# HerreraKrachTeichmann/NJODE

Measured on AMD Instinct MI355X. Metric: paths/sec (training step) on 20k Black-Scholes, 100 steps, higher is better.
Workload: dtype f32; 1 GPU; BlackScholes 20000 paths/GPU x 100 grid steps, every rank's paths as one batch, hidden_size=10, 3x(50,50) tanh nets, dropout 0.1, train step = plan+fwd+bwd+Adam; global_batch=20000, n_obs_rows=199470, euler_steps_per_batch=1820212, params=10071, parallelism=dp1

## Files before the change

include/njode_hip.h:

```cpp
#ifndef NJODE_HIP_H
#define NJODE_HIP_H

#include <stddef.h>
#include <stdint.h>

#ifdef __cplusplus
extern "C" {
#endif

typedef struct ihipStream_t* njodeStream_t;

#define NJODE_OK 0
#define NJODE_E_UNSUPPORTED 1
#define NJODE_E_BADARG 2
#define NJODE_E_WORKSPACE 3
#define NJODE_E_HIP 4

#define NJODE_ACT_TANH 0
#define NJODE_ACT_RELU 1

#define NJODE_F_MASKED 0x1
#define NJODE_F_INPUT_CURRENT_T 0x2
#define NJODE_F_RESIDUAL 0x4
#define NJODE_F_LOSS_EASY 0x8
// ... 64 lines not shown

int njode_workspace_bytes(const NjodeDims* dims, int32_t batch_size, int32_t n_obs,
                          int32_t n_times, int32_t n_steps, int32_t call_flags,
                          size_t* out);

int njode_plan_flush(void);
int njode_plan_bytes(const NjodeDims* dims, int32_t batch_size, int32_t n_obs,
                     int32_t n_times, int32_t n_steps, int32_t call_flags, size_t* out);
int njode_plan_f32(const NjodeDims* dims, const NjodeBatch* batch, const NjodeSchedule* sched,
                   int32_t call_flags, void* plan, size_t plan_bytes, njodeStream_t stream);


int njode_forward_f32(const NjodeDims* dims, const float* params,
                      const NjodeBatch* batch, const NjodeSchedule* sched,
                      int32_t call_flags, float weight, float dropout_p,
                      uint64_t seed, float* hT, float* loss, float* path_h,
                      float* path_y, void* workspace, size_t workspace_bytes,
                      njodeStream_t stream);

int njode_backward_f32(const NjodeDims* dims, const float* params,
                       const NjodeBatch* batch, const NjodeSchedule* sched,
                       int32_t call_flags, float weight, float dropout_p,
                       uint64_t seed, const float* grad_loss, float* grad_params,
                       void* workspace, size_t workspace_bytes,
                       njodeStream_t stream);

int njode_backward_loss_f32(const NjodeDims* dims, const float* params,
                            const NjodeBatch* batch, const NjodeSchedule* sched,
                            int32_t call_flags, float weight, float dropout_p,
                            uint64_t seed, const float* grad_loss, float* grad_params,
                            float* loss, void* workspace, size_t workspace_bytes,
                            njodeStream_t stream);

int njode_adam_step_f32(float* params, const float* grad, float* exp_avg,
                        float* exp_avg_sq, size_t n, float lr, float beta1,
                        float beta2, float eps, float weight_decay, int32_t step,
                        float grad_scale, njodeStream_t stream);

const char* njode_last_error(void);

int njode_profile_enable(int on);
int njode_profile_read(char* out, size_t cap);

int njode_plan_barrier_failures(void);

const char* njode_build_info(void);


#ifdef __cplusplus
}
#endif
#endif
```

njode_amd/_lib.py:

```python
import ctypes as C
import os

_HERE = os.path.dirname(os.path.abspath(__file__))
LIB_PATH = os.environ.get('NJODE_LIB') or os.path.join(_HERE, 'libnjode_hip.so')

NJODE_OK = 0
E_UNSUPPORTED, E_BADARG, E_WORKSPACE, E_HIP = 1, 2, 3, 4
ACT_TANH, ACT_RELU = 0, 1
F_MASKED, F_INPUT_CURRENT_T, F_RESIDUAL, F_LOSS_EASY, F_USE_RNN = 0x1, 0x2, 0x4, 0x8, 0x10
C_TRAIN, C_GET_LOSS, C_RETURN_PATH, C_SAVE_BWD, C_LOSS_IN_BWD = 0x1, 0x2, 0x4, 0x8, 0x10
C_SCHED_KNOWN, C_SCHED_TAIL = 0x20, 0x40
C_PLAN_READY, C_NEED_HT = 0x80, 0x100
C_ROWS_IN_FWD = 0x400
C_GEN_LOCKSTEP = 0x200
C_PLAN_DEFER = 0x800

EXPORTS = ('njode_supported', 'njode_param_count', 'njode_workspace_bytes',
           'njode_plan_bytes', 'njode_plan_f32', 'njode_plan_flush', 'njode_plan_barrier_failures',
           'njode_forward_f32', 'njode_backward_f32', 'njode_backward_loss_f32',
           'njode_adam_step_f32',
           'njode_last_error', 'njode_build_info', 'njode_profile_enable',
           'njode_profile_read',
           'njode_philox4x32_10', 'njode_generate_paths', 'njode_sample_observations',
           'njode_collate_count', 'njode_collate_fill',
           'njode_selftest_dropout_words', 'njode_debug_plan_stamps')
SDE_MODELS = {'BlackScholes': 0, 'OrnsteinUhlenbeck': 1, 'Heston': 2}


MAX_HIDDEN = 8


class NjodeNet(C.Structure):
    _fields_ = [('n_hidden', C.c_int32), ('width', C.c_int32 * MAX_HIDDEN),
                ('act', C.c_int32 * MAX_HIDDEN)]


class NjodeDims(C.Structure):
    _fields_ = [('input_size', C.c_int32), ('hidden_size', C.c_int32),
                ('output_size', C.c_int32), ('n_hidden', C.c_int32),
                ('width', C.c_int32), ('act', C.c_int32), ('flags', C.c_int32),
                ('per_net', C.c_int32), ('nets', NjodeNet * 3)]


class NjodeSchedule(C.Structure):
    _fields_ = [('n_steps', C.c_int32), ('n_times', C.c_int32),
                ('step_dt', C.c_void_p), ('step_t', C.c_void_p),
                ('k_jump', C.c_void_p), ('time_f32', C.c_void_p),
                ('time_ptr', C.c_void_p)]


class NjodeBatch(C.Structure):
    _fields_ = [('batch_size', C.c_int32), ('n_obs', C.c_int32),
                ('start_X', C.c_void_p), ('X', C.c_void_p), ('M', C.c_void_p),
# ... 32 lines not shown
            'njode_amd: {} not found. The NJ-ODE path has no CPU fallback; build '
            'the gfx950 library first: `python -m njode_amd.build` (needs hipcc).'
            .format(LIB_PATH))
    L = C.CDLL(LIB_PATH)
    vp, i32, f32, u64, sz = C.c_void_p, C.c_int32, C.c_float, C.c_uint64, C.c_size_t
    L.njode_supported.argtypes = [C.POINTER(NjodeDims)]
    L.njode_supported.restype = C.c_int
    L.njode_param_count.argtypes = [C.POINTER(NjodeDims)]
    L.njode_param_count.restype = sz
    L.njode_workspace_bytes.argtypes = [C.POINTER(NjodeDims), i32, i32, i32, i32, i32,
                                        C.POINTER(sz)]
    L.njode_workspace_bytes.restype = C.c_int
    L.njode_plan_bytes.argtypes = [C.POINTER(NjodeDims), i32, i32, i32, i32, i32, C.POINTER(sz)]
    L.njode_plan_bytes.restype = C.c_int
    L.njode_plan_f32.argtypes = [C.POINTER(NjodeDims), C.POINTER(NjodeBatch),
                                 C.POINTER(NjodeSchedule), i32, vp, sz, vp]
    L.njode_plan_f32.restype = C.c_int
    L.njode_plan_flush.argtypes = []
    L.njode_plan_flush.restype = C.c_int
    L.njode_plan_barrier_failures.argtypes = []
    L.njode_plan_barrier_failures.restype = C.c_int
    L.njode_forward_f32.argtypes = [C.POINTER(NjodeDims), vp, C.POINTER(NjodeBatch),
                                    C.POINTER(NjodeSchedule), i32, f32, f32, u64,
                                    vp, vp, vp, vp, vp, sz, vp]
    L.njode_forward_f32.restype = C.c_int
    L.njode_backward_f32.argtypes = [C.POINTER(NjodeDims), vp, C.POINTER(NjodeBatch),
                                     C.POINTER(NjodeSchedule), i32, f32, f32, u64,
                                     vp, vp, vp, sz, vp]
    L.njode_backward_f32.restype = C.c_int
    L.njode_backward_loss_f32.argtypes = [C.POINTER(NjodeDims), vp, C.POINTER(NjodeBatch),
                                          C.POINTER(NjodeSchedule), i32, f32, f32, u64,
                                          vp, vp, vp, vp, sz, vp]
    L.njode_backward_loss_f32.restype = C.c_int
    L.njode_adam_step_f32.argtypes = [vp, vp, vp, vp, sz, f32, f32, f32, f32, f32, i32,
                                      f32, vp]
    L.njode_adam_step_f32.restype = C.c_int
    L.njode_last_error.restype = C.c_char_p
    L.njode_build_info.restype = C.c_char_p
    L.njode_profile_enable.argtypes = [C.c_int]
    L.njode_profile_enable.restype = C.c_int
    L.njode_profile_read.argtypes = [C.c_char_p, sz]
    L.njode_profile_read.restype = C.c_int
    f64 = C.c_double
    L.njode_philox4x32_10.argtypes = [i32, vp, vp, vp, vp]
    L.njode_generate_paths.argtypes = [C.POINTER(NjodeSde), u64, vp, vp, vp]
    L.njode_sample_observations.argtypes = [i32, i32, f64, u64, vp, vp, vp, vp]
    L.njode_collate_count.argtypes = [vp, vp, i32, i32, vp, i32, vp, vp, vp]
    L.njode_collate_fill.argtypes = [vp, vp, i32, i32, i32, vp, i32, vp,
                                     C.POINTER(C.c_int32), i32, vp, vp, vp, vp]
    for name in ('njode_philox4x32_10', 'njode_generate_paths', 'njode_sample_observations',
                 'njode_collate_count', 'njode_collate_fill',
           'njode_selftest_dropout_words', 'njode_debug_plan_stamps'):
        getattr(L, name).restype = C.c_int
    L.njode_selftest_dropout_words.argtypes = [u64, u64, C.c_uint32, C.c_uint32, i32, vp, vp]
    L.njode_selftest_dropout_words.restype = C.c_int
    L.njode_debug_plan_stamps.argtypes = [vp, C.c_int]
    _lib = L
    return L


def check(rc):
    if rc == NJODE_OK:
        return
    msg = lib().njode_last_error().decode('utf-8', 'replace')
    if rc == E_UNSUPPORTED:
        raise NjodeUnsupported(rc, msg)
# ... 20 lines not shown
```

njode_amd/csrc/njode_api.hip:

```cpp
#include <hip/hip_runtime.h>

#include <string.h>
#include <cmath>
#include <cstdarg>
#include <cstdio>
#include <cstdlib>
#include <cstring>

#include <rocprim/rocprim.hpp>

#include "../../include/njode_selftest.h"
#include "njode_error.h"
#include "njode_gen_host.h"
#include "njode_host.h"
#include "njode_plan.h"

using namespace njode;

#define NJ_CFG(ID) namespace njode { const CfgOps* njode_cfg_ops_##ID(); }
#include "_generated_cfgs.inc"
#undef NJ_CFG
typedef const CfgOps* (*CfgGetter)();
static const CfgGetter g_cfgs[] = {
#define NJ_CFG(ID) njode::njode_cfg_ops_##ID,
// ... 148 lines not shown
  double total = 288.0e9;
  int dev = 0;
  if (hipGetDevice(&dev) == hipSuccess && dev >= 0 && dev < 16) {
    std::lock_guard<std::mutex> lk(mu);
    if (total_of_dev[dev] == 0.0) {
      size_t fr = 0, tot = 0;
      total_of_dev[dev] = (hipMemGetInfo(&fr, &tot) == hipSuccess && tot > 0) ? (double)tot : 288.0e9;
    }
    total = total_of_dev[dev];
  }
  const double cap = total / 8.0, want = (env_gb > 0.0 ? env_gb : 16.0) * 1.0e9;
  return want < cap ? want : cap;
}
}

namespace {

inline int cdiv(int a, int b) { return (a + b - 1) / b; }
inline int bits_for(unsigned v) {
  int b = 1;
  while (b < 32 && (v >> b)) ++b;
  return b;
}

constexpr int SUM_BLOCKS = 64;
constexpr int RED_SPLIT = 32;

constexpr int PLAN_CS_SMALL_BLOCKS = 32;
struct Layout {
  size_t total = 0;
  size_t len_hist = 0, dense = 0, dense_cells = 0;
  size_t sched, PT, frag, trash, t_of_row, iota, path_sorted, row_by_path, first3, item4, sort_key,
      key_sorted, order, tail4, base_s, h0row, h0start, h_end, lam_end, g_h0, lam_start, loss_terms,
      traj, slab, red_partial, sum_partial, sort_tmp, lk_lam, lk_src, lk_rows, lk_hstart, base16, act, dbits, dbits_row, lk_act, lk_jact, lk_delta, lk_seg, item_pack, tile_last, vflag, cs_small, tile_q, plan_end;
  size_t sort_tmp_bytes = 0;
  int n_waves = 0;
  int n_waves_lock = 0;
  int slab_rows = 0;
  int q4_pt = 16;
  int chain = 0;
  size_t take(size_t bytes) {
    size_t off = total;
    total += (bytes + 255) & ~(size_t)255;
    return off;
  }
};

static int q4_paths_per_tile(int B, double rec_bytes_per_tile = 0.0) {
  static const int env = getenv("NJODE_LOCK4_PT") ? atoi(getenv("NJODE_LOCK4_PT")) : 0;
  if (env == 1 || env == 2 || env == 4 || env == 8 || env == 16) return env;
  int pt = 1;
  while (pt < 16 && (B + pt - 1) / pt > 256) pt *= 2;
  if (rec_bytes_per_tile > 0.0) {
    const double budget = record_budget_bytes();
    while (pt < 16 && (double)((B + pt - 1) / pt) * rec_bytes_per_tile > budget) pt *= 2;
  }
  return pt;
}
static bool chain_paths(const CfgOps* o, int B, int K, int call_flags) {
  static const int bmax = getenv("NJODE_CHAIN_MAX") ? atoi(getenv("NJODE_CHAIN_MAX")) : (1 << 30);
  if (!o->lock_chain || B > bmax) return false;
  if ((call_flags & NJODE_C_RETURN_PATH) && (call_flags & NJODE_C_TRAIN)) return false;
  if (call_flags & NJODE_C_SAVE_BWD) {
    const double rec = (double)B * (K > 0 ? K : 1) * (CHAIN_ACT_FLOATS * 4.0 + 16.0);
    if (rec > record_budget_bytes()) return false;
  }
  return true;
// ... 106 lines not shown
  }
  L.slab_rows = cdiv(n_obs + B, 16) + 128;
  if (L.slab_rows > SLAB_ROWS_MAX) L.slab_rows = SLAB_ROWS_MAX;
  if (L.slab_rows < L.n_waves) L.slab_rows = L.n_waves;
  if (L.slab_rows < L.n_waves_lock) L.slab_rows = L.n_waves_lock;
  if (L.slab_rows < 576) L.slab_rows = 576;
  L.q4_pt = q4_paths_per_tile(B, q4_rec_bytes_per_tile(o, K, call_flags));
  L.chain = chain_paths(o, B, K, call_flags) ? 1 : 0;
  if (L.chain && (call_flags & NJODE_C_TRAIN)) {
    L.dbits = L.take(((size_t)B * (K > 0 ? K : 1) + 1) * 16);
    L.dbits_row = L.take((nr * 3 + nb) * 16);
  }
  if (call_flags & NJODE_C_SAVE_BWD) {
    L.traj = L.take(((size_t)B * (K + 1) + 1) * H * 4);
    L.lk_lam = L.take(((size_t)B * K + 1) * H * 4);
    L.lk_src = L.take(((size_t)B * K + 1) * 4);
    L.lk_rows = L.take(nr * (size_t)(4 * DO + H) * 4);
    L.lk_hstart = L.take(nb * H * 4);
    L.slab = L.take((size_t)L.slab_rows * o->P * 4);
    L.red_partial = L.take((size_t)RED_SPLIT * o->P * 4);
    const bool seg_possible = !(o->dims.flags & (NJODE_F_MASKED | NJODE_F_USE_RNN)) &&
                              !(call_flags & NJODE_C_RETURN_PATH) && (call_flags & NJODE_C_GET_LOSS) &&
                              !((call_flags & NJODE_C_SCHED_KNOWN) && (call_flags & NJODE_C_SCHED_TAIL));
    const size_t act_fl = seg_chain_items(o, B, n_obs, K, call_flags) && CHAIN_ACT_FLOATS > o->act_floats ? CHAIN_ACT_FLOATS : o->act_floats;
    L.act = (o->act_floats > 0 && seg_possible && n_obs > 0)
                ? L.take(((size_t)B * K + 16 * ((size_t)K + 1)) * act_fl * 4) : 0;
    static const bool pack_on = !(getenv("NJODE_ITEM_PACK") && atoi(getenv("NJODE_ITEM_PACK")) == 0);
    L.item_pack = L.tile_last = 0;
    if (L.act && pack_on) {
      const size_t packf = 4 + 4 * (size_t)((1 + D + 3) / 4);
      L.item_pack = L.take((size_t)cdiv((int)nr, 16) * 16 * packf * 4);
      L.tile_last = L.take((size_t)cdiv((int)nr, 16) * 8);
    }
    const int q4pt = L.q4_pt;
    if (L.chain) {
      L.lk_act = L.take(((size_t)B * (K > 0 ? K : 1)) * CHAIN_ACT_FLOATS * 4);
      L.lk_jact = L.take(nr * (size_t)CHAIN_JACT_FLOATS * 4);
    } else {
    L.lk_act = (o->lock_act_floats > 0 && !(call_flags & NJODE_C_RETURN_PATH)) ? L.take((size_t)cdiv(B, q4pt) * (K > 0 ? K : 1) * o->lock_act_floats * 4) : 0;
    static_assert(Q4_JACT_FLOATS == 3 * 2 * 4 * 4, "jump-activation record: 3 evaluations x 2 layers x 4 registers x 4 lane groups");
    L.lk_jact = L.lk_act ? L.take(nr * 4 * (size_t)Q4_JACT_FLOATS * 4) : 0;
    }
    if (!L.chain && L.lk_act && (call_flags & NJODE_C_TRAIN)) {
      L.dbits = L.take((size_t)cdiv(B, q4pt) * (K > 0 ? K : 1) * 256);
      L.dbits_row = L.take(nr * 3 * 4 * 4);
    }
    static const bool store_delta = !(getenv("NJODE_CHAIN_DELTA") && atoi(getenv("NJODE_CHAIN_DELTA")) == 0);
    L.lk_delta = 0;
    if (store_delta && (L.chain || (L.act && seg_chain_items(o, B, n_obs, K, call_flags)))) {
      const double both = (double)B * (K > 0 ? K : 1) * (2.0 * CHAIN_ACT_FLOATS * 4.0 + 16.0);
      if (both <= record_budget_bytes()) L.lk_delta = L.take(((size_t)B * (K > 0 ? K : 1)) * CHAIN_ACT_FLOATS * 4);
    }
    L.lk_seg = (L.lk_delta && o->dims.width < 64) ? L.take((nr + nb) * (size_t)CHAIN_ACT_FLOATS * 4) : 0;
  } else {
    L.traj = L.slab = L.red_partial = L.lk_lam = L.lk_src = L.lk_rows = L.lk_hstart = 0;
    L.act = L.lk_act = L.lk_jact = L.lk_delta = L.lk_seg = L.item_pack = L.tile_last = 0;
  }
  return L;
}

__global__ void k_row_time(const int* __restrict__ time_ptr, int n_times, int n_obs,
                           int* __restrict__ t_of_row, int* __restrict__ iota, int K,
                           int* __restrict__ len_hist, const int* __restrict__ obs_idx, int B,
                           int* __restrict__ dense) {
  if (blockIdx.x == 0)
    for (int s = threadIdx.x; s <= K; s += blockDim.x) len_hist[s] = 0;
  const int r = blockIdx.x * blockDim.x + threadIdx.x;
  if (r >= n_obs) return;
  int lo = 0, hi = n_times;
  while (hi - lo > 1) {
    const int mid = (lo + hi) >> 1;
    if (time_ptr[mid] <= r) lo = mid; else hi = mid;
  }
  t_of_row[r] = lo;
  iota[r] = r;
  if (dense) dense[(size_t)lo * B + obs_idx[r]] = r;
}

__global__ void k_validate_rows(const int* __restrict__ obs_idx, int n_obs, int B,
                                const int* __restrict__ t_of_row, const int* __restrict__ dense,
                                const int* __restrict__ n_obs_ot, int* __restrict__ flag) {
  const int r = blockIdx.x * blockDim.x + threadIdx.x;
  if (r >= n_obs) return;
  const int b = obs_idx[r];
  int bad = 0;
  if (b < 0 || b >= B) bad |= 1;
  else {
    if (dense && dense[(size_t)t_of_row[r] * B + b] != r) bad |= 2;
    if (n_obs_ot && n_obs_ot[b] <= 0) bad |= 4;
// ... 663 lines not shown
    static const int ns_b_env = getenv("NJODE_SPLIT_BWD_BLOCKS") ? atoi(getenv("NJODE_SPLIT_BWD_BLOCKS")) : 32;
    static const int ns_f_env = getenv("NJODE_SPLIT_FWD_BLOCKS") ? atoi(getenv("NJODE_SPLIT_FWD_BLOCKS")) : 96;
    const int n_tiles = cdiv(n_obs > 0 ? n_obs : 1, 16);
    if (n_tiles <= 384) {
      a.n_split_blocks = a.n_blocks_bwd = n_tiles;
    } else {
      static const bool queue_on = getenv("NJODE_BWD_QUEUE") && atoi(getenv("NJODE_BWD_QUEUE")) != 0;
      static const int tot_b_env = getenv("NJODE_BWD_BLOCKS") ? atoi(getenv("NJODE_BWD_BLOCKS")) : 0;
      const int tot_b = tot_b_env > 0 ? tot_b_env : (queue_on ? 2 * device_cus() : 1024);
      a.tile_q_on = queue_on ? 1 : 0;
      a.n_split_blocks = ns_b_env;
      int nsb = tot_b - ns_b_env;
      if (nsb > cdiv(n_tiles, 4)) nsb = cdiv(n_tiles, 4);
      if (a.n_split_blocks + nsb > c.L.slab_rows) nsb = c.L.slab_rows - a.n_split_blocks;
      a.n_blocks_bwd = a.n_split_blocks + nsb;
    }
    if (n_tiles <= 768) {
      a.n_split_fwd = a.n_blocks_fwd = n_tiles;
    } else {
      a.n_split_fwd = ns_f_env;
      static const int tot_f = getenv("NJODE_FWD_BLOCKS") ? atoi(getenv("NJODE_FWD_BLOCKS")) : 3072;
      int nsb = tot_f - ns_f_env;
      if (nsb > cdiv(n_tiles, 4)) nsb = cdiv(n_tiles, 4);
      a.n_blocks_fwd = a.n_split_fwd + nsb;
    }
  }
  {
    static const bool env_fused = getenv("NJODE_ENC_FUSED") && atoi(getenv("NJODE_ENC_FUSED")) != 0;
    a.enc_fused = (env_fused && c.seg && c.ode == ODE_MFMA && a.ode_split && a.n_split_fwd < a.n_blocks_fwd) ? 1 : 0;
  }
  a.n_waves_rows = a.n_waves;
  a.seg_chain = (c.seg && c.ode == ODE_MFMA && a.ode_split && c.o->seg_mfma && seg_chain_items(c.o, B, n_obs, K, call_flags)) ? 1 : 0;
  if (a.seg_chain) a.enc_fused = 0;
  {
    static const bool fuse = !(getenv("NJODE_DW_ENC_FUSED") && atoi(getenv("NJODE_DW_ENC_FUSED")) == 0);
    a.dw_enc_fused = (fuse && a.seg_chain && a.cdelta && a.cseg && a.dw_pair_blocks > 0 && dims->width < 64) ? 1 : 0;
  }
  return NJODE_OK;
}

int upload_schedule(const Call& c, const NjodeSchedule* s, void* ws, hipStream_t st) {
  const int K = s->n_steps, nt = s->n_times;
  char* dst = (char*)ws + c.L.sched;
  const size_t bdt = (size_t)K * 4, bt = (size_t)nt * 4, bp = ((size_t)nt + 1) * 4;
  const char* h0 = (const char*)s->step_dt;
  const bool contiguous = K > 0 && nt > 0 && (const char*)s->step_t == h0 + bdt &&
                          (const char*)s->k_jump == h0 + 2 * bdt &&
                          (const char*)s->time_f32 == h0 + 2 * bdt + bt &&
                          (const char*)s->time_ptr == h0 + 2 * bdt + 2 * bt;
  if (contiguous) {
    HIP_TRY(hipMemcpyAsync(dst, h0, 2 * bdt + 2 * bt + bp, hipMemcpyHostToDevice, st));
  } else {
    if (K > 0) {
      HIP_TRY(hipMemcpyAsync(dst, s->step_dt, bdt, hipMemcpyHostToDevice, st));
      HIP_TRY(hipMemcpyAsync(dst + bdt, s->step_t, bdt, hipMemcpyHostToDevice, st));
    }
    if (nt > 0) {
      HIP_TRY(hipMemcpyAsync(dst + 2 * bdt, s->k_jump, bt, hipMemcpyHostToDevice, st));
      HIP_TRY(hipMemcpyAsync(dst + 2 * bdt + bt, s->time_f32, bt, hipMemcpyHostToDevice, st));
    }
    HIP_TRY(hipMemcpyAsync(dst + 2 * bdt + 2 * bt, s->time_ptr, bp, hipMemcpyHostToDevice, st));
  }
  return NJODE_OK;
}

__global__ void __launch_bounds__(1024) k_sum_small(const float* __restrict__ x, int n,
// ... 571 lines not shown
        k_reduce_slabs_stage2_sum<<<nbx + 1, 256, 0, st>>>(partial, d.P, grad_loss, grad_params, sp, nbx, loss);
      } else {
        if (loss_pending) sum_to(c, workspace, c.a.n_obs, loss, st);
        k_reduce_slabs_stage1<<<dim3(nbx, RED_SPLIT), 256, 0, st>>>(c.a.slab, d, partial);
        k_reduce_slabs_stage2<<<nbx, 256, 0, st>>>(partial, d.P, grad_loss, grad_params);
      }
    }
  }
  HIP_TRY(hipGetLastError());
  return NJODE_OK;
}

extern "C" int njode_backward_f32(const NjodeDims* dims, const float* params,
                                  const NjodeBatch* batch, const NjodeSchedule* sched,
                                  int32_t call_flags, float weight, float dropout_p,
                                  uint64_t seed, const float* grad_loss, float* grad_params,
                                  void* workspace, size_t workspace_bytes,
                                  njodeStream_t stream) {
  return backward_impl(dims, params, batch, sched, call_flags, weight, dropout_p, seed, grad_loss,
                       grad_params, nullptr, workspace, workspace_bytes, stream);
}

extern "C" int njode_backward_loss_f32(const NjodeDims* dims, const float* params,
                                       const NjodeBatch* batch, const NjodeSchedule* sched,
                                       int32_t call_flags, float weight, float dropout_p,
                                       uint64_t seed, const float* grad_loss, float* grad_params,
                                       float* loss, void* workspace, size_t workspace_bytes,
                                       njodeStream_t stream) {
  if (!loss) return fail(NJODE_E_BADARG, "null loss pointer");
  return backward_impl(dims, params, batch, sched, call_flags, weight, dropout_p, seed, grad_loss,
                       grad_params, loss, workspace, workspace_bytes, stream);
}

extern "C" int njode_adam_step_f32(float* params, const float* grad, float* exp_avg,
                                   float* exp_avg_sq, size_t n, float lr, float beta1,
                                   float beta2, float eps, float weight_decay, int32_t step,
                                   float grad_scale, njodeStream_t stream) {
  if (!params || !grad || !exp_avg || !exp_avg_sq) return fail(NJODE_E_BADARG, "null argument");
  if (step < 1) return fail(NJODE_E_BADARG, "step must be >= 1");
  if (n == 0) return NJODE_OK;
  const double c1 = 1.0 - pow((double)beta1, (double)step);
  const double c2 = 1.0 - pow((double)beta2, (double)step);
  k_adam<<<(unsigned)((n + 255) / 256), 256, 0, (hipStream_t)stream>>>(
      params, grad, exp_avg, exp_avg_sq, n, (float)(lr / c1), beta1, beta2, eps, weight_decay,
      (float)(1.0 / sqrt(c2)), grad_scale);
  HIP_TRY(hipGetLastError());
  return NJODE_OK;
}

namespace {
__global__ void k_selftest_dropout_words(njode::DropCtx dc, unsigned long long gid, uint32_t tkey,
                                         uint32_t net, int n_words, uint32_t* out) {
  const int g = threadIdx.x;
  if (g >= 4) return;
  uint32_t st = njode::drop_state(dc, (uint32_t)gid, (uint32_t)(gid >> 32) + 0x5bd1e995u * (g + 1),
                                  tkey, net);
  for (int i = 0; i < n_words; ++i) out[g * n_words + i] = njode::xs32(st);
}
}

extern "C" int njode_selftest_dropout_words(uint64_t seed, uint64_t path_id, uint32_t time_key,
                                            uint32_t net, int32_t n_words, uint32_t* out_words,
                                            void* stream) {
  if (!out_words || n_words <= 0) return fail(NJODE_E_BADARG, "null output / n_words <= 0");
  njode::DropCtx dc;
  dc.seed_lo = (uint32_t)seed;
// ... 9 lines not shown
```

njode_amd/csrc/njode_cfg.hip:

```cpp
#include <cstdlib>
#include <cstring>

#include "njode_host.h"
#if NJ_PART >= 4
#include "njode_chain.h"
#include "njode_chain_seg.h"
#include "njode_chain_dw.h"
#endif

#define NJ_CAT_(a, b) a##b
#define NJ_CAT(a, b) NJ_CAT_(a, b)

namespace njode {

#ifndef NJ_RNN
#define NJ_RNN 0
#endif
using C = Cfg<NJ_D, NJ_H, NJ_DO, NJ_NH, NJ_W, NJ_ACT, (NJ_MASKED != 0), (NJ_CURT != 0),
              (NJ_RES != 0), (NJ_RNN != 0)>;

static inline int cdiv(int a, int b) { return (a + b - 1) / b; }

hipError_t NJ_CAT(njode_seg_forward_, NJ_ID)(const KArgs& a, bool drop, bool tails, int ode,
                                            hipStream_t st);
// ... 60 lines not shown
    if constexpr (SegChainOk<C>::value) {
      if (a.seg_chain) {
        seg_chain_bits_body<C>(a, (int)blockIdx.x - n_pack, (int)gridDim.x - n_pack);
        return;
      }
    }
    if constexpr (HAS_SPLIT) {
      const int nb = (int)gridDim.x - n_pack;
      drop_bits_tile_steps<C>(a, ((int)blockIdx.x - n_pack) * 4 + (threadIdx.x >> 6), nb * 4);
    }
  }
}

template <class CC> static void launch_pack_frags(const KArgs& a, hipStream_t st, bool bits = false) {
  if constexpr (HAS_MFMA) {
    using ES = typename EncS<CC>::type;
    using DS = typename DecS<CC>::type;
    const int n_pack = cdiv((2 * MF<CC>::NALL + ES::NALL + DS::NALL) * 64, 256);
    if (bits) {
      const long long work = a.seg_chain ? (long long)a.K * a.B / 64 + 1
                                         : (long long)cdiv(a.n_obs, 16) * cdiv(a.K > 0 ? a.K : 1, 8);
      const int nb = (int)(work / 4 + 1 < 1024 ? work / 4 + 1 : 1024);
      k_pack_all_bits<CC, ES, DS><<<n_pack + nb, 256, 0, st>>>(a, n_pack);
    } else {
      k_pack_all<CC, ES, DS><<<n_pack, 256, 0, st>>>(a.P, a.frag, a.frag2, a.frag_enc, a.frag_dec, a.dc.inv_keep,
                                                  a.plan_sync_zero);
    }
  }
}
template <class CC, bool DROP> static void launch_mfma_enc(const KArgs& a, hipStream_t st) {
  if constexpr (HAS_MFMA) {
    const int n_tiles = cdiv(a.n_obs + a.B, 16);
    static const int enc_blocks = getenv("NJODE_ENC_BLOCKS") ? atoi(getenv("NJODE_ENC_BLOCKS")) : 4096;
    k_encode_rows_mfma<CC, DROP><<<n_tiles < enc_blocks ? n_tiles : enc_blocks, 64, 0, st>>>(a);
  }
}
template <class CC, bool DROP> static void launch_mfma_jump(const KArgs& a, hipStream_t st) {
  if constexpr (HAS_MFMA) {
    const int n_tiles = cdiv(a.n_obs, 16);
    k_jump_rows_mfma<CC, DROP><<<n_tiles < 2048 ? n_tiles : 2048, 64, 0, st>>>(a);
  }
}
template <class CC, bool DROP> static void launch_ode_bwd_mfma(const KArgs& a, bool split, hipStream_t st) {
  if constexpr (HAS_MFMA) {
    if constexpr (HAS_SPLIT) {
      if (split) {
        ProfScope ps("k_ode_bwd_mixed", st);
        if (a.tile_q_on) k_ode_bwd_mixed<CC, DROP, true><<<a.n_blocks_bwd, 256, 0, st>>>(a);
        else k_ode_bwd_mixed<CC, DROP, false><<<a.n_blocks_bwd, 256, 0, st>>>(a);
        return;
      }
    }
    ProfScope ps("k_ode_bwd_mfma", st);
    k_ode_bwd_mfma<CC, DROP><<<a.n_waves_ode / 4, 256, 0, st>>>(a);
  }
}
template <class CC, bool DROP> static void launch_jump_rows_bwd(const KArgs& a, hipStream_t st) {
  if constexpr (HAS_MFMA) {
    ProfScope ps("k_jump_rows_bwd_mfma", st);
    k_jump_rows_bwd_mfma<CC, DROP><<<a.n_waves_rows / 4, 256, 0, st>>>(a);
  }
}
template <class CC, bool DROP>
static void launch_mfma_rows_bwd(const KArgs& a, bool split, hipStream_t st) {
  if constexpr (HAS_MFMA) {
    if (a.defer_loss != 2) launch_jump_rows_bwd<CC, DROP>(a, st);
    bool enc_done = false;
// ... 458 lines not shown
```

njode_amd/csrc/njode_kernels.h:

```cpp
#pragma once
#include "njode_device.h"

namespace njode {

constexpr uint32_t NET_ODE = 0, NET_ENC = 1, NET_DEC = 2, NET_DEC_BJ = 3, NET_DEC_ROW = 4;
constexpr uint32_t TKEY_START = 0xffffffffu;

template <int D_, int H_, int DO_, int NH_, int W_, int ACT_, bool MASKED_, bool CURT_,
          bool RES_, bool RNN_ = false>
struct Cfg {
  static constexpr int D = D_, H = H_, DO = DO_, NH = NH_, W = (NH_ > 0 ? W_ : 1), ACT = ACT_;
  static constexpr bool MASKED = MASKED_, CURT = CURT_, RES = RES_, RNN = RNN_;
  static constexpr int ODE_IN = D + H + (CURT ? 3 : 2);
  static constexpr int ENC_IN = MASKED ? 2 * D : D;
  using Ode = NetL<ODE_IN, H, NH, W_>;
  using Enc = NetL<ENC_IN, H, NH, W_>;
  using Dec = NetL<H, DO, NH, W_>;
  static constexpr int OFF_ODE = 0, OFF_ENC = Ode::SIZE, OFF_DEC = Ode::SIZE + Enc::SIZE;
  static constexpr int OFF_GRU = OFF_DEC + Dec::SIZE;
  static constexpr int G_WIH = 0, G_WHH = 3 * H * D, G_BIH = G_WHH + 3 * H * H, G_BHH = G_BIH + 3 * H;
  static constexpr int GRU_SIZE = G_BHH + 3 * H;
  static constexpr int P = OFF_GRU + (RNN ? GRU_SIZE : 0);
  static_assert(!(RNN && MASKED), "the GRU jump is not defined for masked models");
  static constexpr int ENC_CASE = !RES ? 0 : (D <= H ? 1 : 2);
// ... 62 lines not shown
  float* g_hstart;
  float* lact;
  float* jact;
  float* loss_terms;
  float* slab;
  float* trash;
  int* tile_q;
  int tile_q_on;
  int n_waves;
  int n_waves_ode;
  int n_waves_rows;
  const float* g_hT;
  float* hT;
  float* path_h;
  float* path_y;
  float weight;
  int loss_easy;
  int want_path, want_loss;
  int save_traj;
  int defer_loss;
  int ode_split;
  int n_split_blocks, n_blocks_bwd, n_split_fwd, n_blocks_fwd;
  int q4_pt;
  int chain;
  int seg_chain;
  float* cdelta;
  float* cseg;
  float* item_pack;
  long long* tile_last;
  int dw_pair_blocks, dw_seg_blocks;
  int dw_enc_fused;
  unsigned* plan_sync_zero;
  int enc_fused;
  DropCtx dc;
  float keep;
};

template <class C, bool TWO = (C::NH == 2)> struct ChainOk { static constexpr bool value = false; };
template <class C> struct ChainOk<C, true> {
  static constexpr bool value =
      C::MASKED && !C::RNN && C::W <= 64 && C::H <= 64 && C::D <= 64 && C::DO <= 64 && C::D == C::DO &&
      (C::ENC_CASE == 0 || (C::ENC_CASE == 1 && C::D == C::H)) &&
      (C::DEC_CASE == 0 || (C::DEC_CASE == 1 && C::DO == C::H));
};
template <class C, bool TWO = (C::NH == 2)> struct SegChainOk { static constexpr bool value = false; };
template <class C> struct SegChainOk<C, true> {
  static constexpr bool value = !C::MASKED && !C::RNN && C::W <= 64 && C::W > 16 && C::H <= 16 && C::D <= 8;
};
constexpr int CHAIN_MAX_WAVES = 8;
constexpr int CHAIN_ACT_FLOATS = 2 * 64;
constexpr int CHAIN_JACT_FLOATS = 3 * 2 * 64;

template <int N> NJ_DEV void load_vec(const float* p, float (&v)[N]) {
#pragma unroll
  for (int i = 0; i < N; ++i) v[i] = p[i];
}
template <int N> NJ_DEV void store_vec(float* p, const float (&v)[N]) {
#pragma unroll
  for (int i = 0; i < N; ++i) p[i] = v[i];
}
NJ_DEV int wave_max(int v) {
#pragma unroll
  for (int o = 32; o > 0; o >>= 1) v = max(v, __shfl_xor(v, o));
  return v;
}

// ... 590 lines not shown
```

njode_amd/csrc/njode_mfma_rows.h:

```cpp
#pragma once
#include "njode_mfma.h"

namespace njode {

template <int IN_, int OUT_, int W_> struct MS {
  static constexpr int IN = IN_, OUT = OUT_, W = W_;
  static constexpr int Q0 = (IN + 1 + 3) / 4, Q1 = (W + 1 + 3) / 4;
  static constexpr int QO = (OUT + 3) / 4, QW = (W + 3) / 4, QI = (IN + 3) / 4;
  static constexpr int MT1 = (W + 15) / 16, MTO = (OUT + 15) / 16, MTI = (IN + 15) / 16;
  static constexpr int NT1 = (W + 1 + 15) / 16, NT0 = (IN + 1 + 15) / 16;
  static constexpr int F1 = 0, F2 = F1 + MT1 * Q0, F3 = F2 + MT1 * Q1, NFWD = F3 + MTO * Q1;
  static constexpr int B3 = NFWD, B2 = B3 + MT1 * QO, B1 = B2 + MT1 * QW, NALL = B1 + MTI * QW;
  static constexpr int ET = EdgeRows<W>::TILE, ER = EdgeRows<W>::R;
  static constexpr int G2M = ER ? ET : MT1, G2N = ER ? ET : NT1;
};

template <class NL, class S>
NJ_DEV void pack_net_value(const float* __restrict__ Pn, float* __restrict__ frag, int idx) {
  if (idx >= S::NALL * 64) return;
  const int f = idx >> 6, l = idx & 63, g = l >> 4, c = l & 15;
  const float *W1 = Pn + NL::woff(0), *b1 = Pn + NL::boff(0), *W2 = Pn + NL::woff(1),
              *b2 = Pn + NL::boff(1), *W3 = Pn + NL::woff(2), *b3 = Pn + NL::boff(2);
  float v = 0.0f;
  if (f < S::F2) {
// ... 358 lines not shown
NJ_DEV void fill_by_group(float (&dq)[NQ], const float (&v)[N], int g) {
  if constexpr (Q < NQ) {
    dq[Q] = by_group<Q, N>(v, g);
    fill_by_group<NQ, N, Q + 1>(dq, v, g);
  }
}

template <class C> struct EncS { using type = MS<C::ENC_IN, C::H, C::W>; };
template <class C> struct DecS { using type = MS<C::H, C::DO, C::W>; };

template <class C, class S>
NJ_DEV void enc_input(const float* xp, float (&b0)[S::Q0], int g) {
#pragma unroll
  for (int q = 0; q < S::Q0; ++q) {
    const int u = 4 * q + g;
    const float xv = xp[u < C::D ? u : 0];
    b0[q] = u < C::D ? tanh_f(xv) : (u == C::D ? 1.0f : 0.0f);
  }
}
template <class C> NJ_DEV float enc_residual(const float* xp, int u) {
  if constexpr (C::ENC_CASE == 1) {
    return xp[u % C::D];
  } else if constexpr (C::ENC_CASE == 2) {
    constexpr int mult = C::D / C::H;
    float s = 0.0f;
#pragma unroll
    for (int cc = 0; cc < mult; ++cc) s += xp[cc * C::H + (u < C::H ? u : 0)];
    return s * (1.0f / mult);
  } else {
    return 0.0f;
  }
}

template <class C, bool DROP>
__global__ void __launch_bounds__(64) k_encode_rows_mfma(KArgs a) {
  using S = typename EncS<C>::type;
  const int lane = threadIdx.x, g = lane >> 4, c = lane & 15;
  FwdFrags<S> F;
  F.load(a.frag_enc, lane);
  const int total = a.n_obs + a.B;
  const int n_tiles = (total + 15) / 16;
  float* const trash = a.trash + lane * C::H;
  for (int tile = blockIdx.x; tile < n_tiles; tile += gridDim.x) {
    const int t0 = tile * 16 + c;
    const bool valid = t0 < total;
    const int tid = valid ? t0 : 0;
    const bool is_row = tid < a.n_obs;
    const int b = is_row ? a.obs_idx[tid] : tid - a.n_obs;
    const float* xp = is_row ? a.X + (size_t)tid * C::D : a.start_X + (size_t)b * C::D;
    float b0[S::Q0], a1[S::Q1], a2[S::Q1];
    enc_input<C, S>(xp, b0, g);
    uint32_t k1, k2;
    row_keep_bits<DROP>(a, a.gid0 + b, is_row ? (uint32_t)a.k_jump[a.t_of_row[tid]] : TKEY_START,
                        NET_ENC, g, S::Q1, k1, k2);
    f32x4 out[S::MTO];
    mnet_fwd<S, C::ACT, DROP>(F, b0, a1, a2, out, k1, k2, a.dc.inv_keep, g);
    float* dstrow = valid ? (is_row ? a.h0row + (size_t)tid * C::H : a.h0start + (size_t)b * C::H)
                          : trash;
#pragma unroll
    for (int q = 0; q < S::QO; ++q) {
      const int u = 4 * q + g;
      const float v = out[q / 4][q % 4] + enc_residual<C>(xp, u < C::H ? u : 0);
      float* dst = u < C::H ? dstrow + u : trash;
      *dst = v;
    }
  }
}

template <class C, bool DROP>
__global__ void __launch_bounds__(64) k_encode_rows_items(KArgs a, int n_path_tiles) {
  using S = typename EncS<C>::type;
  const int lane = threadIdx.x, g = lane >> 4, c = lane & 15;
  FwdFrags<S> F;
  F.load(a.frag_enc, lane);
  const int T = (int)a.base_s[a.K + 2];
  const int n_tiles = n_path_tiles + (a.n_obs > 0 ? T : 0);
  float* const trash = a.trash + lane * C::H;
  for (int tile = blockIdx.x; tile < n_tiles; tile += gridDim.x) {
    bool valid, is_row;
    int b, row;
    if (tile < n_path_tiles) {
      b = tile * 16 + c;
      valid = b < a.B;
      b = valid ? b : 0;
      row = a.last_row[b];
      is_row = row >= 0;
    } else {
      const int j = (tile - n_path_tiles) * 16 + c;
      valid = j < a.n_obs;
      const int r = a.order[valid ? j : 0];
      b = a.obs_idx[r];
      row = a.item_prev[r];
      is_row = row >= 0;
    }
    const int rr = is_row ? row : 0;
    const float* xp = is_row ? a.X + (size_t)rr * C::D : a.start_X + (size_t)b * C::D;
    float b0[S::Q0], a1[S::Q1], a2[S::Q1];
    enc_input<C, S>(xp, b0, g);
    uint32_t k1, k2;
// ... 179 lines not shown
  static_assert(3 * GradTiles<S>::NG * 256 <= 4 * 2 * IMG_FLOATS + S::NALL * 64, "tile reduction does not fit");
  if (G.reduce_block((lfp)lds_raw, wv, lane))
    G.template flush<NL>(a.slab + (size_t)blockIdx.x * C::P + C::OFF_DEC, g, c);
}

template <class C> struct EncBwdLds {
  static constexpr int FLOATS = 4 * 2 * IMG_FLOATS + EncS<C>::type::NALL * 64;
};
template <class C, bool DROP>
NJ_DEV void encode_rows_bwd_body(const KArgs& a, float* lds_raw, int block, int n_blocks) {
  using S = typename EncS<C>::type;
  using NL = typename C::Enc;
  const int lane = threadIdx.x & 63, wv = threadIdx.x >> 6, g = lane >> 4, c = lane & 15;
  const int wave = block * 4 + wv, n_waves = n_blocks * 4;
  lfp img_d = (lfp)lds_raw + wv * 2 * IMG_FLOATS, img_a = img_d + IMG_FLOATS;
  lfp fimg = (lfp)lds_raw + 4 * 2 * IMG_FLOATS;
  LdsFrags<S>::stage(fimg, a.frag_enc, threadIdx.x, 256);
  for (int i = threadIdx.x; i < 4 * 2 * IMG_FLOATS; i += 256) lds_raw[i] = 0.0f;
  __syncthreads();
  LdsFrags<S> F;
  F.init(fimg, lane);
  LdsFrags<S>& Bf = F;
  GradTiles<S> G;
  G.zero();
  const int total = a.n_obs + a.B;
  const int n_tiles = (total + 15) / 16;
  for (int tile = wave; tile < n_tiles; tile += n_waves) {
    const int t0 = tile * 16 + c;
    const bool valid = t0 < total;
    const int tid = valid ? t0 : 0;
    const bool is_row = tid < a.n_obs;
    const int b = is_row ? a.obs_idx[tid] : tid - a.n_obs;
    const float* xp = is_row ? a.X + (size_t)tid * C::D : a.start_X + (size_t)b * C::D;
    const int nxt = is_row ? a.item_next[tid] : a.first_row[b];
    const int nx = nxt >= 0 ? nxt : 0, rr = is_row ? tid : 0;
    float gh[S::QO];
#pragma unroll
    for (int q = 0; q < S::QO; ++q) {
      const int u = 4 * q + g, uu = u < C::H ? u : 0;
      const float l = a.lam_start[(size_t)nx * C::H + uu];
      const float p = a.g_h0[(size_t)rr * C::H + uu];
      gh[q] = (valid && u < C::H) ? ((nxt >= 0 ? l : 0.0f) + (is_row ? p : 0.0f)) : 0.0f;
    }
    float b0[S::Q0], a1[S::Q1], a2[S::Q1];
    enc_input<C, S>(xp, b0, g);
    uint32_t k1, k2;
    row_keep_bits<DROP>(a, a.gid0 + b, is_row ? (uint32_t)a.k_jump[a.t_of_row[tid]] : TKEY_START,
                        NET_ENC, g, S::Q1, k1, k2);
    f32x4 out[S::MTO], din[1];
    mnet_fwd<S, C::ACT, DROP>(F, b0, a1, a2, out, k1, k2, a.dc.inv_keep, g);
    mnet_bwd<S, C::ACT, DROP, false>(Bf, G, img_d, img_a, gh, b0, a1, a2, k1, k2, a.dc.inv_keep,
                                     a.keep, din, g, c);
  }
  static_assert(3 * GradTiles<S>::NG * 256 <= 4 * 2 * IMG_FLOATS + S::NALL * 64, "tile reduction does not fit");
  if (G.reduce_block((lfp)lds_raw, wv, lane))
    G.template flush<NL>(a.slab + (size_t)block * C::P + C::OFF_ENC, g, c);
}
template <class C, bool DROP>
__global__ void __launch_bounds__(256, 2) k_encode_rows_bwd_mfma(KArgs a) {
  __shared__ __attribute__((aligned(16))) float lds_raw[EncBwdLds<C>::FLOATS];
  encode_rows_bwd_body<C, DROP>(a, lds_raw, (int)blockIdx.x, (int)gridDim.x);
}

}
```

njode_amd/models.py:

```python
import ctypes
import os

import numpy as np
import torch

from . import _lib
from .schedule import PinnedRing, ScheduleCache


def init_weights(m, bias=0.0):
    if type(m) == torch.nn.Linear:
        torch.nn.init.xavier_uniform_(m.weight)
        if m.bias is not None:
            m.bias.data.fill_(bias)


def save_checkpoint(model, optimizer, path, epoch):
    if not os.path.exists(path):
        os.makedirs(path)
    torch.save({'epoch': epoch, 'weight': model.weight,
                'model_state_dict': model.state_dict(),
                'optimizer_state_dict': optimizer.state_dict()},
               os.path.join(path, 'checkpt.tar'))


def get_ckpt_model(ckpt_path, model, optimizer, device):
    ckpt_path = os.path.join(ckpt_path, 'checkpt.tar')
    if not os.path.exists(ckpt_path):
        raise Exception("Checkpoint " + ckpt_path + " does not exist.")
    checkpt = torch.load(ckpt_path, map_location='cpu', weights_only=False)
    if optimizer is not None:
        optimizer.load_state_dict(checkpt['optimizer_state_dict'])
    model.load_state_dict(checkpt['model_state_dict'])
    model.epoch = checkpt['epoch']
    model.weight = checkpt['weight']
    model.to(device)


def _norm(t, dim=1, eps=1e-10):
    return torch.sqrt(torch.sum(t, dim=dim) + eps)
# ... 717 lines not shown

    def _forward_via_op(self, times, time_ptr, X, obs_idx, delta_t, T, start_X, n_obs_ot,
                        get_loss, until_T, M, want_grad):
        from . import ops
        self._ensure_flat()
        hT, loss, _ = torch.ops.njode_amd.forward(
            list(self._flat_params), start_X, X, obs_idx, n_obs_ot if get_loss else None,
            M if self.masked else None, torch.as_tensor(np.asarray(times, dtype=np.float64)),
            torch.as_tensor(np.asarray(time_ptr, dtype=np.int64)), float(delta_t), float(T),
            ops.register_model(self), bool(get_loss), bool(until_T), bool(want_grad))
        if not get_loss:
            return hT, 0
        loss_out = loss.reshape(())
        if not self.device_outputs:
            loss_out = loss_out.cpu()
        return hT, loss_out

    def loss_and_grad(self, times, time_ptr, X, obs_idx, delta_t, T, start_X, n_obs_ot,
                      M=None, plan=None):
        grad = self.flat_grad()
        dev = start_X.device
        stream = torch.cuda.current_stream(dev)
        call, sched, slot_i, B = self._make_call(
            times, time_ptr, X, obs_idx, delta_t, T, start_X, n_obs_ot, False, True, False,
            M, save_bwd=True, plan_key=(obs_idx, time_ptr), want_hT=self.masked or self.use_rnn, plan=plan,
            stream=stream)
        loss = (self.loss_slot() if self.dp_loss_in_bucket
                else torch.empty(1, dtype=torch.float32, device=dev))
        hT = (torch.empty(B, self.hidden_size, dtype=torch.float32, device=dev)
              if self.masked or self.use_rnn else None)
        call.flags |= _lib.C_LOSS_IN_BWD
        self._last_stream = stream
        try:
            self._run_forward(call, hT, loss, None, None, slot_i, stream)
            if self._ones is None or self._ones.device != dev:
                self._ones = torch.ones(1, dtype=torch.float32, device=dev)
            self._run_backward(call, self._ones, grad, loss=loss, stream=stream)
        finally:
            self._release_ws(call)
        return hT, loss.reshape(())

    def evaluate(self, times, time_ptr, X, obs_idx, delta_t, T, start_X, n_obs_ot,
                 stockmodel, cond_exp_fun_kwargs=None,
                 diff_fun=lambda x, y: np.mean((x - y) ** 2), return_paths=False, M=None):
        self.eval()
        _, _, path_t, path_h, path_y = self.forward(
            times, time_ptr, X, obs_idx, delta_t, T, start_X, None, return_path=True,
            get_loss=False, until_T=True, M=M)
        _, true_path_t, true_path_y = stockmodel.compute_cond_exp(
            times, time_ptr, X.detach().cpu().numpy(), obs_idx.detach().cpu().numpy(),
            delta_t, T, start_X.detach().cpu().numpy(), n_obs_ot.detach().cpu().numpy(),
            return_path=True, get_loss=False)
        eval_loss = diff_fun(path_y.detach().cpu().numpy(), true_path_y)
        if return_paths:
            return eval_loss, path_t, true_path_t, path_y, true_path_y
        return eval_loss

    def get_pred(self, times, time_ptr, X, obs_idx, delta_t, T, start_X, M=None):
        self.eval()
        _, _, path_t, path_h, path_y = self.forward(
            times, time_ptr, X, obs_idx, delta_t, T, start_X, None, return_path=True,
            get_loss=False, until_T=True, M=M)
        if not self.device_outputs:
            path_y = path_y.cpu()
        return {'pred': path_y, 'pred_t': path_t}


class FusedAdam:

    def __init__(self, model, lr=1e-3, betas=(0.9, 0.999), eps=1e-8, weight_decay=0.0,
# ... 100 lines not shown
```

Baseline: 23.75 million paths/s.

## Store encoder dropout bits in forward for reuse in backward; add one-call loss-and-grad entry

The encoder forward kernel now writes its per-lane dropout keep masks into a new workspace buffer. The encoder backward reads those masks instead of regenerating them with the Philox-based row_keep_bits. A new njode_loss_and_grad_f32 entry point runs forward and backward in a single ctypes call, cutting Python-side launch overhead, and the encoder kernels gain a waves_per_eu attribute. The cost is extra workspace and global memory traffic for the bits, and the fused call path is taken only when hT is not needed.

```diff
diff --git a/include/njode_hip.h b/include/njode_hip.h
--- a/include/njode_hip.h
+++ b/include/njode_hip.h
@@ -120,6 +120,13 @@
                             float* loss, void* workspace, size_t workspace_bytes,
                             njodeStream_t stream);
 
+int njode_loss_and_grad_f32(const NjodeDims* dims, const float* params,
+                            const NjodeBatch* batch, const NjodeSchedule* sched,
+                            int32_t call_flags, float weight, float dropout_p,
+                            uint64_t seed, const float* grad_loss, float* grad_params,
+                            float* loss, void* workspace, size_t workspace_bytes,
+                            njodeStream_t stream);
+
 int njode_adam_step_f32(float* params, const float* grad, float* exp_avg,
                         float* exp_avg_sq, size_t n, float lr, float beta1,
                         float beta2, float eps, float weight_decay, int32_t step,
diff --git a/njode_amd/_lib.py b/njode_amd/_lib.py
--- a/njode_amd/_lib.py
+++ b/njode_amd/_lib.py
@@ -18,7 +18,7 @@
 EXPORTS = ('njode_supported', 'njode_param_count', 'njode_workspace_bytes',
            'njode_plan_bytes', 'njode_plan_f32', 'njode_plan_flush', 'njode_plan_barrier_failures',
            'njode_forward_f32', 'njode_backward_f32', 'njode_backward_loss_f32',
-           'njode_adam_step_f32',
+           'njode_loss_and_grad_f32', 'njode_adam_step_f32',
            'njode_last_error', 'njode_build_info', 'njode_profile_enable',
            'njode_profile_read',
            'njode_philox4x32_10', 'njode_generate_paths', 'njode_sample_observations',
@@ -117,6 +117,8 @@
                                           C.POINTER(NjodeSchedule), i32, f32, f32, u64,
                                           vp, vp, vp, vp, sz, vp]
     L.njode_backward_loss_f32.restype = C.c_int
+    L.njode_loss_and_grad_f32.argtypes = L.njode_backward_loss_f32.argtypes
+    L.njode_loss_and_grad_f32.restype = C.c_int
     L.njode_adam_step_f32.argtypes = [vp, vp, vp, vp, sz, f32, f32, f32, f32, f32, i32,
                                       f32, vp]
     L.njode_adam_step_f32.restype = C.c_int
diff --git a/njode_amd/csrc/njode_api.hip b/njode_amd/csrc/njode_api.hip
--- a/njode_amd/csrc/njode_api.hip
+++ b/njode_amd/csrc/njode_api.hip
@@ -204,7 +204,7 @@
   size_t len_hist = 0, dense = 0, dense_cells = 0;
   size_t sched, PT, frag, trash, t_of_row, iota, path_sorted, row_by_path, first3, item4, sort_key,
       key_sorted, order, tail4, base_s, h0row, h0start, h_end, lam_end, g_h0, lam_start, loss_terms,
-      traj, slab, red_partial, sum_partial, sort_tmp, lk_lam, lk_src, lk_rows, lk_hstart, base16, act, dbits, dbits_row, lk_act, lk_jact, lk_delta, lk_seg, item_pack, tile_last, vflag, cs_small, tile_q, plan_end;
+      traj, slab, red_partial, sum_partial, sort_tmp, lk_lam, lk_src, lk_rows, lk_hstart, base16, act, dbits, dbits_row, lk_act, lk_jact, lk_delta, lk_seg, item_pack, tile_last, enc_bits, vflag, cs_small, tile_q, plan_end;
   size_t sort_tmp_bytes = 0;
   int n_waves = 0;
   int n_waves_lock = 0;
@@ -377,6 +377,10 @@
       L.item_pack = L.take((size_t)cdiv((int)nr, 16) * 16 * packf * 4);
       L.tile_last = L.take((size_t)cdiv((int)nr, 16) * 8);
     }
+    static const bool enc_bits_on = !(getenv("NJODE_ENC_BITS") && atoi(getenv("NJODE_ENC_BITS")) == 0);
+    L.enc_bits = (enc_bits_on && o->seg_mfma && seg_possible && n_obs > 0 && (call_flags & NJODE_C_TRAIN) &&
+                  nr + nb < ((size_t)1 << 30))
+                     ? L.take((size_t)cdiv((int)(nr + nb), 16) * 64 * 4) : 0;
     const int q4pt = L.q4_pt;
     if (L.chain) {
       L.lk_act = L.take(((size_t)B * (K > 0 ? K : 1)) * CHAIN_ACT_FLOATS * 4);
@@ -399,7 +403,7 @@
     L.lk_seg = (L.lk_delta && o->dims.width < 64) ? L.take((nr + nb) * (size_t)CHAIN_ACT_FLOATS * 4) : 0;
   } else {
     L.traj = L.slab = L.red_partial = L.lk_lam = L.lk_src = L.lk_rows = L.lk_hstart = 0;
-    L.act = L.lk_act = L.lk_jact = L.lk_delta = L.lk_seg = L.item_pack = L.tile_last = 0;
+    L.act = L.lk_act = L.lk_jact = L.lk_delta = L.lk_seg = L.item_pack = L.tile_last = L.enc_bits = 0;
   }
   return L;
 }
@@ -1129,6 +1133,8 @@
   a.n_waves_rows = a.n_waves;
   a.seg_chain = (c.seg && c.ode == ODE_MFMA && a.ode_split && c.o->seg_mfma && seg_chain_items(c.o, B, n_obs, K, call_flags)) ? 1 : 0;
   if (a.seg_chain) a.enc_fused = 0;
+  a.enc_bits = (c.L.enc_bits && c.seg && c.drop && c.ode == ODE_MFMA && c.o->seg_mfma && !a.enc_fused)
+                   ? (uint32_t*)(w + c.L.enc_bits) : nullptr;
   {
     static const bool fuse = !(getenv("NJODE_DW_ENC_FUSED") && atoi(getenv("NJODE_DW_ENC_FUSED")) == 0);
     a.dw_enc_fused = (fuse && a.seg_chain && a.cdelta && a.cseg && a.dw_pair_blocks > 0 && dims->width < 64) ? 1 : 0;
@@ -1766,6 +1772,20 @@
                        grad_params, loss, workspace, workspace_bytes, stream);
 }
 
+extern "C" int njode_loss_and_grad_f32(const NjodeDims* dims, const float* params,
+                                       const NjodeBatch* batch, const NjodeSchedule* sched,
+                                       int32_t call_flags, float weight, float dropout_p,
+                                       uint64_t seed, const float* grad_loss, float* grad_params,
+                                       float* loss, void* workspace, size_t workspace_bytes,
+                                       njodeStream_t stream) {
+  if (!loss) return fail(NJODE_E_BADARG, "null loss pointer");
+  const int rc = njode_forward_f32(dims, params, batch, sched, call_flags, weight, dropout_p, seed, nullptr,
+                                   loss, nullptr, nullptr, workspace, workspace_bytes, stream);
+  if (rc) return rc;
+  return backward_impl(dims, params, batch, sched, call_flags, weight, dropout_p, seed, grad_loss,
+                       grad_params, loss, workspace, workspace_bytes, stream);
+}
+
 extern "C" int njode_adam_step_f32(float* params, const float* grad, float* exp_avg,
                                    float* exp_avg_sq, size_t n, float lr, float beta1,
                                    float beta2, float eps, float weight_decay, int32_t step,
diff --git a/njode_amd/csrc/njode_cfg.hip b/njode_amd/csrc/njode_cfg.hip
--- a/njode_amd/csrc/njode_cfg.hip
+++ b/njode_amd/csrc/njode_cfg.hip
@@ -116,7 +116,8 @@
   if constexpr (HAS_MFMA) {
     const int n_tiles = cdiv(a.n_obs + a.B, 16);
     static const int enc_blocks = getenv("NJODE_ENC_BLOCKS") ? atoi(getenv("NJODE_ENC_BLOCKS")) : 4096;
-    k_encode_rows_mfma<CC, DROP><<<n_tiles < enc_blocks ? n_tiles : enc_blocks, 64, 0, st>>>(a);
+    if (DROP && a.enc_bits) k_encode_rows_mfma_bits<CC, DROP><<<n_tiles < enc_blocks ? n_tiles : enc_blocks, 64, 0, st>>>(a);
+    else k_encode_rows_mfma<CC, DROP><<<n_tiles < enc_blocks ? n_tiles : enc_blocks, 64, 0, st>>>(a);
   }
 }
 template <class CC, bool DROP> static void launch_mfma_jump(const KArgs& a, hipStream_t st) {
diff --git a/njode_amd/csrc/njode_kernels.h b/njode_amd/csrc/njode_kernels.h
--- a/njode_amd/csrc/njode_kernels.h
+++ b/njode_amd/csrc/njode_kernels.h
@@ -118,6 +118,7 @@
   int dw_enc_fused;
   unsigned* plan_sync_zero;
   int enc_fused;
+  uint32_t* enc_bits;
   DropCtx dc;
   float keep;
 };
diff --git a/njode_amd/csrc/njode_mfma_rows.h b/njode_amd/csrc/njode_mfma_rows.h
--- a/njode_amd/csrc/njode_mfma_rows.h
+++ b/njode_amd/csrc/njode_mfma_rows.h
@@ -414,8 +414,8 @@
   }
 }
 
-template <class C, bool DROP>
-__global__ void __launch_bounds__(64) k_encode_rows_mfma(KArgs a) {
+template <class C, bool DROP, bool BITS>
+NJ_DEV void encode_rows_fwd_body(const KArgs& a) {
   using S = typename EncS<C>::type;
   const int lane = threadIdx.x, g = lane >> 4, c = lane & 15;
   FwdFrags<S> F;
@@ -435,6 +435,7 @@
     uint32_t k1, k2;
     row_keep_bits<DROP>(a, a.gid0 + b, is_row ? (uint32_t)a.k_jump[a.t_of_row[tid]] : TKEY_START,
                         NET_ENC, g, S::Q1, k1, k2);
+    if constexpr (DROP && BITS) a.enc_bits[(unsigned)tile * 64u + (unsigned)lane] = k1 | (k2 << 16);
     f32x4 out[S::MTO];
     mnet_fwd<S, C::ACT, DROP>(F, b0, a1, a2, out, k1, k2, a.dc.inv_keep, g);
     float* dstrow = valid ? (is_row ? a.h0row + (size_t)tid * C::H : a.h0start + (size_t)b * C::H)
@@ -447,6 +448,15 @@
       *dst = v;
     }
   }
+}
+
+template <class C, bool DROP>
+__global__ void __launch_bounds__(64) __attribute__((amdgpu_waves_per_eu(4, 4))) k_encode_rows_mfma(KArgs a) {
+  encode_rows_fwd_body<C, DROP, false>(a);
+}
+template <class C, bool DROP>
+__global__ void __launch_bounds__(64) __attribute__((amdgpu_waves_per_eu(4, 4))) k_encode_rows_mfma_bits(KArgs a) {
+  encode_rows_fwd_body<C, DROP, true>(a);
 }
 
 template <class C, bool DROP>
@@ -692,6 +702,9 @@
     const bool is_row = tid < a.n_obs;
     const int b = is_row ? a.obs_idx[tid] : tid - a.n_obs;
     const float* xp = is_row ? a.X + (size_t)tid * C::D : a.start_X + (size_t)b * C::D;
+    const bool stored = DROP && a.enc_bits != nullptr;
+    uint32_t kw = 0;
+    if (stored) kw = a.enc_bits[(unsigned)tile * 64u + (unsigned)lane];
     const int nxt = is_row ? a.item_next[tid] : a.first_row[b];
     const int nx = nxt >= 0 ? nxt : 0, rr = is_row ? tid : 0;
     float gh[S::QO];
@@ -705,8 +718,13 @@
     float b0[S::Q0], a1[S::Q1], a2[S::Q1];
     enc_input<C, S>(xp, b0, g);
     uint32_t k1, k2;
-    row_keep_bits<DROP>(a, a.gid0 + b, is_row ? (uint32_t)a.k_jump[a.t_of_row[tid]] : TKEY_START,
-                        NET_ENC, g, S::Q1, k1, k2);
+    if (stored) {
+      k1 = kw & 0xffffu;
+      k2 = kw >> 16;
+    } else {
+      row_keep_bits<DROP>(a, a.gid0 + b, is_row ? (uint32_t)a.k_jump[a.t_of_row[tid]] : TKEY_START,
+                          NET_ENC, g, S::Q1, k1, k2);
+    }
     f32x4 out[S::MTO], din[1];
     mnet_fwd<S, C::ACT, DROP>(F, b0, a1, a2, out, k1, k2, a.dc.inv_keep, g);
     mnet_bwd<S, C::ACT, DROP, false>(Bf, G, img_d, img_a, gh, b0, a1, a2, k1, k2, a.dc.inv_keep,
diff --git a/njode_amd/models.py b/njode_amd/models.py
--- a/njode_amd/models.py
+++ b/njode_amd/models.py
@@ -6,6 +6,8 @@
 
 from . import _lib
 from .schedule import PinnedRing, ScheduleCache
+
+_ONE_CALL_STEP = os.environ.get('NJODE_ONE_CALL_STEP', '1') != '0'
 
 
 def init_weights(m, bias=0.0):
@@ -789,10 +791,19 @@
         call.flags |= _lib.C_LOSS_IN_BWD
         self._last_stream = stream
         try:
-            self._run_forward(call, hT, loss, None, None, slot_i, stream)
             if self._ones is None or self._ones.device != dev:
                 self._ones = torch.ones(1, dtype=torch.float32, device=dev)
-            self._run_backward(call, self._ones, grad, loss=loss, stream=stream)
+            if hT is None and _ONE_CALL_STEP:
+                rc = _lib.lib().njode_loss_and_grad_f32(
+                    ctypes.byref(call.dims), self._flat.data_ptr(), ctypes.byref(call.batch),
+                    ctypes.byref(call.sched), call.flags, call.weight, call.p_drop, call.seed,
+                    self._ones.data_ptr(), grad.data_ptr(), loss.data_ptr(), call.ws.data_ptr(),
+                    call.ws.numel(), stream.cuda_stream)
+                self._release_slots(slot_i, stream)
+                _lib.check(rc)
+            else:
+                self._run_forward(call, hT, loss, None, None, slot_i, stream)
+                self._run_backward(call, self._ones, grad, loss=loss, stream=stream)
         finally:
             self._release_ws(call)
         return hT, loss.reshape(())
```

New measurement: 23.48 million paths/s. -1.1%, worse.
